# nilsfriess/dune-ddm

Measured on AMD Instinct MI355X. Metric: preconditioned CG iterations/sec (two-level additive Schwarz), 3D Poisson 10M DoF, higher is better.
Workload: dtype f64

## Files before the change

dune-ddm_amd/csrc/kernels.hpp:

```cpp
#pragma once
#include <hip/hip_runtime.h>
#include <stdint.h>

namespace ddm {

constexpr int WG = 256;
constexpr int SPMV_NNZ = 2048;
constexpr int RED_MAX_BLOCKS = 1024;
constexpr int RED_TRIPS = 4;

__device__ __forceinline__ int xcd_remap(int orig, int nwg)
{
  const int q = nwg >> 3, r = nwg & 7, xcd = orig & 7;
  return (xcd < r ? xcd * (q + 1) : r * (q + 1) + (xcd - r) * q) + (orig >> 3);
}

__device__ __forceinline__ double wave_sum(double v)
{
#pragma unroll
  for (int o = 32; o > 0; o >>= 1) v += __shfl_down(v, o, 64);
  return v;
}

__device__ __forceinline__ double block_sum(double v, double *lds4)
// ... 923 lines not shown
    }
    if (stamp) {
      asm volatile("s_waitcnt vmcnt(0)" ::: "memory");
      DDM_STAMP(t_gather)
    }
    const double out = upper ? s * s0 : s;
    if (act) {
      if (wt) st_sc1(x + row, out);
      else x[row] = out;
    }
    if (H.level_done) {
      asm volatile("s_waitcnt vmcnt(0)" ::: "memory");
      if (lane == 0) {
        unsigned *f = flags + H.flag_base + rank;
        if (wt) __hip_atomic_store(f, epoch, __ATOMIC_RELAXED, __HIP_MEMORY_SCOPE_AGENT);
        else *(volatile unsigned *)f = epoch;
      }
    }
    DDM_STAMP(t_drain)
    n_items += 1;
  }
  if (stamp && lane == 0) {
    stamps[0] = t_tile;
    stamps[1] = t_poll;
    stamps[2] = t_gather;
    stamps[3] = t_drain;
    stamps[4] = n_items;
    stamps[5] = __builtin_amdgcn_s_memtime() - t_begin;
  }
#undef DDM_STAMP
}

__global__ void k_w_permute_in(int64_t n, const int64_t *__restrict__ lpos, const int32_t *__restrict__ rows, const double *__restrict__ d,
                               double *__restrict__ dperm)
{
  for (int64_t i = blockIdx.x * (int64_t)WG + threadIdx.x; i < n; i += (int64_t)gridDim.x * WG) dperm[lpos[i]] = d[rows[lpos[i]]];
}
__global__ void k_w_permute_out(int64_t n, const int64_t *__restrict__ upos, const int32_t *__restrict__ rows, const double *__restrict__ xp,
                                double *__restrict__ x)
{
  for (int64_t i = blockIdx.x * (int64_t)WG + threadIdx.x; i < n; i += (int64_t)gridDim.x * WG) x[rows[upos[i]]] = xp[upos[i]];
}

__global__ void k_perm_gather(int64_t n, int nrhs, const int32_t *__restrict__ perm, const double *__restrict__ src, int64_t ld, double *__restrict__ dst)
{
  const int64_t tot = n * nrhs;
  for (int64_t t = blockIdx.x * (int64_t)WG + threadIdx.x; t < tot; t += (int64_t)gridDim.x * WG) {
    const int64_t i = t / nrhs;
    dst[t] = src[(int64_t)perm[i] * ld + (t - i * nrhs)];
  }
}
__global__ void k_perm_scatter(int64_t n, int nrhs, const int32_t *__restrict__ perm, const double *__restrict__ src, double *__restrict__ dst, int64_t ld)
{
  const int64_t tot = n * nrhs;
  for (int64_t t = blockIdx.x * (int64_t)WG + threadIdx.x; t < tot; t += (int64_t)gridDim.x * WG) {
    const int64_t i = t / nrhs;
    dst[(int64_t)perm[i] * ld + (t - i * nrhs)] = src[t];
  }
}
__global__ void k_perm_scatter_add(int64_t n, int nrhs, const int32_t *__restrict__ perm, const double *__restrict__ src, double *__restrict__ dst, int64_t ld)
{
  const int64_t tot = n * nrhs;
  for (int64_t t = blockIdx.x * (int64_t)WG + threadIdx.x; t < tot; t += (int64_t)gridDim.x * WG) {
    const int64_t i = t / nrhs;
    dst[(int64_t)perm[i] * ld + (t - i * nrhs)] += src[t];
  }
}
__global__ __launch_bounds__(WG) void k_residual_rowmajor(int64_t n, int nrhs, const int64_t *__restrict__ rp, const int32_t *__restrict__ ci, const double *__restrict__ va,
                                                          const double *__restrict__ x, int64_t ldx, const double *__restrict__ d, int64_t ldd, double *__restrict__ r, int64_t ldr)
{
  const int64_t t = (int64_t)blockIdx.x * WG + threadIdx.x;
  const int64_t row = t / nrhs;
  if (row >= n) return;
  const int j = (int)(t - row * nrhs);
  double s = d[row * ldd + j];
  for (int64_t k = rp[row]; k < rp[row + 1]; ++k) s -= va[k] * x[(int64_t)ci[k] * ldx + j];
  r[row * ldr + j] = s;
}
__global__ void k_extend(int64_t n, const int32_t *__restrict__ ext_map, const double *__restrict__ d, double *__restrict__ dov)
{
  for (int64_t i = blockIdx.x * (int64_t)WG + threadIdx.x; i < n; i += (int64_t)gridDim.x * WG) {
    const int32_t m = ext_map[i];
    dov[i] = m >= 0 ? d[m] : 0.0;
  }
}
template <bool ACC, bool SCALE>
__global__ void k_restrict(int64_t n, const int32_t *__restrict__ ext_map, const double *__restrict__ xov,
                           const double *__restrict__ w, double *__restrict__ x)
{
  for (int64_t i = blockIdx.x * (int64_t)WG + threadIdx.x; i < n; i += (int64_t)gridDim.x * WG) {
    const int32_t m = ext_map[i];
    if (m >= 0) {
      const double v = SCALE ? xov[i] * w[i] : xov[i];
      x[m] = ACC ? x[m] + v : v;
    }
  }
}
__global__ void k_scale(int64_t n, const double *__restrict__ w, double *__restrict__ x)
{
  for (int64_t i = blockIdx.x * (int64_t)WG + threadIdx.x; i < n; i += (int64_t)gridDim.x * WG) x[i] *= w[i];
}
__global__ void k_fill(int64_t n, double v, double *__restrict__ x)
{
  for (int64_t i = blockIdx.x * (int64_t)WG + threadIdx.x; i < n; i += (int64_t)gridDim.x * WG) x[i] = v;
}
__global__ void k_axpy(int64_t n, double a, const double *__restrict__ x, double *__restrict__ y)
{
  for (int64_t i = blockIdx.x * (int64_t)WG + threadIdx.x; i < n; i += (int64_t)gridDim.x * WG) y[i] += a * x[i];
}

__global__ void k_axpy_negdev(int64_t n, const double *__restrict__ h, const double *__restrict__ x, double *__restrict__ y)
{
  const double a = h[0];
  for (int64_t i = blockIdx.x * (int64_t)WG + threadIdx.x; i < n; i += (int64_t)gridDim.x * WG) y[i] -= a * x[i];
}
__global__ void k_scal(int64_t n, double a, double *__restrict__ x)
{
  for (int64_t i = blockIdx.x * (int64_t)WG + threadIdx.x; i < n; i += (int64_t)gridDim.x * WG) x[i] *= a;
}

__global__ void k_pack(int64_t n, const int64_t *__restrict__ idx, const double *__restrict__ v, double *__restrict__ buf)
{
  for (int64_t i = blockIdx.x * (int64_t)WG + threadIdx.x; i < n; i += (int64_t)gridDim.x * WG) buf[i] = v[idx[i]];
}
template <bool ADD>
__global__ void k_unpack(int64_t ndst, const int64_t *__restrict__ dst_idx, const int64_t *__restrict__ dst_ptr,
                         const int64_t *__restrict__ src_pos, const double *__restrict__ buf, double *__restrict__ v)
{
  for (int64_t t = blockIdx.x * (int64_t)WG + threadIdx.x; t < ndst; t += (int64_t)gridDim.x * WG) {
    const int64_t i = dst_idx[t];
    double s = ADD ? v[i] : 0.0;
    for (int64_t k = dst_ptr[t]; k < dst_ptr[t + 1]; ++k) s = ADD ? s + buf[src_pos[k]] : buf[src_pos[k]];
    v[i] = s;
  }
}

template <bool MASKED>
__global__ __launch_bounds__(WG) void k_dot_partial(int64_t n, const uint8_t *__restrict__ mask, const double *__restrict__ x,
                                                     const double *__restrict__ y, double *__restrict__ partial)
{
  __shared__ double red[4];
  double s = 0.0;
  const int64_t step = (int64_t)gridDim.x * WG;
  int64_t i = blockIdx.x * (int64_t)WG + threadIdx.x;
  for (; i + (RED_TRIPS - 1) * step < n; i += RED_TRIPS * step) {
    double a[RED_TRIPS], b[RED_TRIPS];
    bool own[RED_TRIPS];
#pragma unroll
    for (int u = 0; u < RED_TRIPS; ++u) a[u] = x[i + u * step], b[u] = y[i + u * step], own[u] = !MASKED || mask[i + u * step];
#pragma unroll
    for (int u = 0; u < RED_TRIPS; ++u)
      if (own[u]) s += a[u] * b[u];
  }
  for (; i < n; i += step)
    if (!MASKED || mask[i]) s += x[i] * y[i];
  s = block_sum(s, red);
  if (threadIdx.x == 0) partial[blockIdx.x] = s;
}
__global__ __launch_bounds__(WG) void k_reduce_final(int nb, const double *__restrict__ partial, double *__restrict__ out)
{
  __shared__ double red[4];
  double s = 0.0;
  for (int i = threadIdx.x; i < nb; i += WG) s += partial[i];
  s = block_sum(s, red);
  if (threadIdx.x == 0) out[0] = s;
}

__global__ void k_cg_lambda(double *scal) { scal[2] = scal[0] / scal[1]; }
__global__ void k_cg_beta(double *scal)
{
  scal[4] = scal[3] / scal[0];
  scal[0] = scal[3];
}
__global__ void k_cg_update(int64_t n, const double *__restrict__ scal, const double *__restrict__ p,
                            const double *__restrict__ q, double *__restrict__ x, double *__restrict__ b)
{
  const double lam = scal[2];
  for (int64_t i = blockIdx.x * (int64_t)WG + threadIdx.x; i < n; i += (int64_t)gridDim.x * WG) {
    x[i] += lam * p[i];
    b[i] -= lam * q[i];
  }
}
template <bool MASKED>
__global__ __launch_bounds__(WG) void k_cg_update_norm(int64_t n, const double *__restrict__ scal, const uint8_t *__restrict__ mask,
                                                        const double *__restrict__ p, const double *__restrict__ q, double *__restrict__ x,
                                                        double *__restrict__ b, double *__restrict__ partial)
{
  __shared__ double red[4];
  const double lam = scal[2];
  double s = 0.0;
  for (int64_t i = blockIdx.x * (int64_t)WG + threadIdx.x; i < n; i += (int64_t)gridDim.x * WG) {
    x[i] += lam * p[i];
    const double bi = b[i] - lam * q[i];
    b[i] = bi;
    if (!MASKED || mask[i]) s += bi * bi;
  }
  s = block_sum(s, red);
  if (threadIdx.x == 0) partial[blockIdx.x] = s;
}
__global__ void k_cg_direction(int64_t n, const double *__restrict__ scal, const double *__restrict__ q, double *__restrict__ p)
{
  const double beta = scal[4];
  for (int64_t i = blockIdx.x * (int64_t)WG + threadIdx.x; i < n; i += (int64_t)gridDim.x * WG) p[i] = beta * p[i] + q[i];
}

static constexpr int COARSE_KMAX = 256;
struct RowChunk {
  int64_t r0, r1;
  int32_t sub, pad;
};
__global__ __launch_bounds__(WG) void k_coarse_restrict_partial(int kmax, int64_t ld, const double *__restrict__ basis,
                                                                 const double *__restrict__ d, const RowChunk *__restrict__ chunks,
                                                                 double *__restrict__ partial , int nchunk)
{
  for (int ch = blockIdx.x; ch < nchunk; ch += gridDim.x) {
  const RowChunk c = chunks[ch];
  const int lane = threadIdx.x & 63, w = threadIdx.x >> 6;
  for (int j = w; j < kmax; j += 4) {
    const double *bj = basis + (int64_t)j * ld;
    double s = 0.0;
    int64_t r = c.r0 + lane;
    for (; r + 7 * 64 < c.r1; r += 8 * 64) {
      double bv[8], dv[8];
#pragma unroll
      for (int u = 0; u < 8; ++u) bv[u] = __builtin_nontemporal_load(bj + r + u * 64);
#pragma unroll
      for (int u = 0; u < 8; ++u) dv[u] = d[r + u * 64];
#pragma unroll
      for (int u = 0; u < 8; ++u) s += bv[u] * dv[u];
    }
    for (; r < c.r1; r += 64) s += bj[r] * d[r];
    s = wave_sum(s);
    if (lane == 0) partial[(int64_t)ch * kmax + j] = s;
  }
  }
}
__global__ __launch_bounds__(WG) void k_coarse_restrict_final(int nsub, int kmax, const int32_t *__restrict__ sub_chunk_ptr,
                                                               const double *__restrict__ partial,
                                                               const int64_t *__restrict__ coarse_index, int64_t K,
                                                               double *__restrict__ d0)
{
  for (int64_t i = threadIdx.x; i < K; i += WG) d0[i] = 0.0;
  __syncthreads();
  for (int t = threadIdx.x; t < nsub * kmax; t += WG) {
    const int s = t / kmax, j = t % kmax;
    const int64_t gi = coarse_index[t];
    if (gi < 0) continue;
    double acc = 0.0;
    for (int c = sub_chunk_ptr[s]; c < sub_chunk_ptr[s + 1]; ++c) acc += partial[(int64_t)c * kmax + j];
    d0[gi] = acc;
  }
}
__global__ __launch_bounds__(WG) void k_dense_mv(int64_t K, const double *__restrict__ M, const double *__restrict__ v,
                                                  double *__restrict__ out)
{
  const int lane = threadIdx.x & 63;
  const int64_t row = blockIdx.x * 4 + (threadIdx.x >> 6);
  if (row >= K) return;
  double s = 0.0;
  for (int64_t c = lane; c < K; c += 64) s += M[row * K + c] * v[c];
  s = wave_sum(s);
  if (lane == 0) out[row] = s;
}
__global__ __launch_bounds__(WG) void k_coarse_prolong(int kmax, int64_t ld, const double *__restrict__ basis,
                                                        const double *__restrict__ x0, const int64_t *__restrict__ coarse_index,
                                                        const RowChunk *__restrict__ chunks, double *__restrict__ xov, int nchunk)
{
  __shared__ double cj[COARSE_KMAX];
  static_assert(COARSE_KMAX <= WG, "one thread per coefficient");
  for (int ch = blockIdx.x; ch < nchunk; ch += gridDim.x) {
  const RowChunk c = chunks[ch];
  __syncthreads();
  if (threadIdx.x < kmax) {
    const int64_t gi = coarse_index[(int64_t)c.sub * kmax + threadIdx.x];
    cj[threadIdx.x] = gi >= 0 ? x0[gi] : 0.0;
  }
  __syncthreads();
  for (int64_t r = c.r0 + threadIdx.x; r < c.r1; r += 2 * WG) {
    const int64_t r2 = r + WG < c.r1 ? r + WG : r;
    double s = 0.0, s2 = 0.0;
    int j = 0;
    for (; j + 4 <= kmax; j += 4) {
      double bv[4], bw[4];
#pragma unroll
      for (int u = 0; u < 4; ++u) bv[u] = __builtin_nontemporal_load(basis + (int64_t)(j + u) * ld + r);
#pragma unroll
      for (int u = 0; u < 4; ++u) bw[u] = __builtin_nontemporal_load(basis + (int64_t)(j + u) * ld + r2);
#pragma unroll
      for (int u = 0; u < 4; ++u) s += cj[j + u] * bv[u];
#pragma unroll
      for (int u = 0; u < 4; ++u) s2 += cj[j + u] * bw[u];
    }
    for (; j < kmax; ++j) {
      s += cj[j] * basis[(int64_t)j * ld + r];
      s2 += cj[j] * basis[(int64_t)j * ld + r2];
    }
    xov[r] = s;
    if (r2 != r) xov[r2] = s2;
  }
  }
}

constexpr int SPREAD_WG = 64;
typedef const __attribute__((address_space(1))) double *uniform_gptr;
__device__ __forceinline__ uniform_gptr uniform_global(const double *p)
{
  const uint64_t v = (uint64_t)p;
  const uint32_t lo = __builtin_amdgcn_readfirstlane((uint32_t)v), hi = __builtin_amdgcn_readfirstlane((uint32_t)(v >> 32));
  return (uniform_gptr)(((uint64_t)hi << 32) | lo);
}
__global__ __launch_bounds__(SPREAD_WG) void k_coarse_restrict_spread(int kmax, int64_t ld, const double *__restrict__ basis,
                                                                       const double *__restrict__ d, const RowChunk *__restrict__ chunks,
                                                                       double *__restrict__ partial , int nchunk)
{
  const int lane = threadIdx.x;
  const int64_t nitem = (int64_t)nchunk * kmax;
  for (int64_t item = blockIdx.x; item < nitem; item += gridDim.x) {
    const int ch = (int)(item / kmax), j = (int)(item % kmax);
    const RowChunk c = chunks[ch];
    const double *bj = basis + (int64_t)j * ld;
    double s = 0.0;
    int64_t r = c.r0 + lane;
    for (; r + 7 * 64 < c.r1; r += 8 * 64) {
      double bv[8], dv[8];
#pragma unroll
      for (int u = 0; u < 8; ++u) bv[u] = __builtin_nontemporal_load(bj + r + u * 64);
#pragma unroll
      for (int u = 0; u < 8; ++u) dv[u] = d[r + u * 64];
#pragma unroll
      for (int u = 0; u < 8; ++u) s += bv[u] * dv[u];
    }
    for (; r < c.r1; r += 64) s += bj[r] * d[r];
    s = wave_sum(s);
    if (lane == 0) partial[item] = s;
  }
}
__global__ __launch_bounds__(SPREAD_WG) void k_coarse_prolong_spread(int kmax, int64_t ld, const double *__restrict__ basis,
                                                                      const double *__restrict__ x0, const int64_t *__restrict__ coarse_index,
                                                                      const RowChunk *__restrict__ chunks, double *__restrict__ xov, int nchunk)
{
  __shared__ double cj[COARSE_KMAX];
  const int lane = threadIdx.x;
  for (int ch = blockIdx.x; ch < nchunk; ch += gridDim.x) {
    const RowChunk c = chunks[ch];
    __syncthreads();
    for (int j = lane; j < kmax; j += SPREAD_WG) {
      const int64_t gi = coarse_index[(int64_t)c.sub * kmax + j];
      cj[j] = gi >= 0 ? x0[gi] : 0.0;
    }
    __syncthreads();
    for (int64_t rb = c.r0; rb < c.r1; rb += 4 * SPREAD_WG) {
      const int nrow = (int)(c.r1 - rb < 4 * SPREAD_WG ? c.r1 - rb : 4 * SPREAD_WG);
      if (lane >= nrow) continue;
      unsigned lo[4];
#pragma unroll
      for (int q = 0; q < 4; ++q) lo[q] = (unsigned)(lane + q * SPREAD_WG < nrow ? lane + q * SPREAD_WG : lane);
      double s[4] = {0.0, 0.0, 0.0, 0.0};
      int j = 0;
#pragma unroll 1
      for (; j + 4 <= kmax; j += 4) {
        double bv[4][4];
#pragma unroll
        for (int u = 0; u < 4; ++u) {
          const uniform_gptr bc = uniform_global(basis + (int64_t)(j + u) * ld + rb);
#pragma unroll
          for (int q = 0; q < 4; ++q) bv[q][u] = __builtin_nontemporal_load(bc + lo[q]);
        }
#pragma unroll
        for (int q = 0; q < 4; ++q)
#pragma unroll
          for (int u = 0; u < 4; ++u) s[q] += cj[j + u] * bv[q][u];
      }
      for (; j < kmax; ++j) {
        const double *bc = basis + (int64_t)j * ld + rb;
#pragma unroll
        for (int q = 0; q < 4; ++q) s[q] += cj[j] * bc[lo[q]];
      }
      xov[rb + lo[0]] = s[0];
#pragma unroll
      for (int q = 1; q < 4; ++q)
        if (lo[q] != (unsigned)lane) xov[rb + lo[q]] = s[q];
    }
  }
}

}
```

dune-ddm_amd/csrc/preconditioners.hpp:

```cpp
#pragma once

static int dot_device(ddm_ctx *ctx, int64_t n, const uint8_t *mask, const double *x, const double *y, double *result_dev)
{
  const int nb = grid_for(n, WG * 4, RED_MAX_BLOCKS);
  if (mask)
    hipLaunchKernelGGL(k_dot_partial<true>, dim3(nb), dim3(WG), 0, ctx->stream, n, mask, x, y, ctx->partial);
  else
    hipLaunchKernelGGL(k_dot_partial<false>, dim3(nb), dim3(WG), 0, ctx->stream, n, mask, x, y, ctx->partial);
  hipLaunchKernelGGL(k_reduce_final, dim3(1), dim3(WG), 0, ctx->stream, nb, ctx->partial, result_dev);
  HIPCHECK(ctx, hipGetLastError());
  DDMCHECK(ctx_allreduce(ctx, result_dev, 1, "scalar product"));
  return DDM_OK;
}

template <class Launch>
static void for_column_groups(int m, Launch &&launch)
{
  for (int c0 = 0; c0 < m;) {
    const int cb = m - c0 >= 8 ? 8 : m - c0 >= 4 ? 4 : m - c0 >= 2 ? 2 : 1;
    launch(c0, cb);
    c0 += cb;
  }
}
#define DDM_MULTI_CB_DISPATCH(KERNEL, MASKED, cb, ...)                                                                 \
// ... 197 lines not shown
                  : ddm_ilu0_create(ctx, A_dir, nblocks, block_ptr, &S->solver));
  DDMCHECK(upload(ctx, ext_map_host, n, S->ext_map));
  if (pou_host) DDMCHECK(upload(ctx, pou_host, n, S->pou));
  if (S->d_ovlp.alloc(n) != hipSuccess || S->x_ovlp.alloc(n) != hipSuccess) return fail(ctx, DDM_EHIP, "alloc");
  *out = S.release();
  return DDM_OK;
}
extern "C" void ddm_schwarz_destroy(ddm_schwarz *S) { delete S; }
extern "C" int64_t ddm_schwarz_num_levels(const ddm_schwarz *S, int upper) { return ddm_ilu0_num_levels(S->solver, upper); }
extern "C" int64_t ddm_schwarz_factor_nnz(const ddm_schwarz *S) { return (S && S->solver) ? S->solver->nnz : 0; }
extern "C" int ddm_schwarz_engine(const ddm_schwarz *S) { return S ? ddm_ilu0_engine(S->solver) : -1; }
extern "C" ddm_ilu0 *ddm_schwarz_local_solver(ddm_schwarz *S) { return S ? S->solver : nullptr; }
extern "C" int ddm_schwarz_status(ddm_ctx *ctx, const ddm_schwarz *S)
{
  if (!S) return fail(ctx, DDM_EINVAL, "ddm_schwarz_status: bad arguments");
  int st = 0;
  DDMCHECK(ddm_ilu0_status(ctx, S->solver, &st));
  if (st) return fail(ctx, DDM_ENUMERIC, "local triangular solve timed out waiting for a dependency (code %d): results are invalid", st);
  return DDM_OK;
}
static int local_status_check(ddm_ctx *ctx, const ddm_schwarz *S)
{
  if (const unsigned e = S ? ilu0_peek_status(S->solver) : 0u)
    return fail(ctx, DDM_ENUMERIC, "an earlier local triangular solve timed out waiting for a dependency (code %u): results since then are invalid", e);
  return DDM_OK;
}
static int schwarz_apply_impl(ddm_ctx *ctx, ddm_schwarz *S, double *x, const double *d, bool acc)
{
  DDMCHECK(local_status_check(ctx, S));
  {
    ScopedTimer t(ctx, "Schwarz/get defect");
    hipLaunchKernelGGL(k_extend, dim3(grid_for(S->n)), dim3(WG), 0, ctx->stream, S->n, S->ext_map, d, S->d_ovlp);
    DDMCHECK(ddm_halo_exchange(ctx, S->copy, S->d_ovlp));
  }
  {
    ScopedTimer t(ctx, "Schwarz/local solve");
    DDMCHECK(ddm_ilu0_solve(ctx, S->solver, S->d_ovlp, S->x_ovlp));
  }
  {
    ScopedTimer t(ctx, "Schwarz/add solution");
    if (S->type == 1 && S->pou)
      hipLaunchKernelGGL(k_scale, dim3(grid_for(S->n)), dim3(WG), 0, ctx->stream, S->n, S->pou, S->x_ovlp);
    DDMCHECK(ddm_halo_exchange(ctx, S->add, S->x_ovlp));
    if (acc)
      hipLaunchKernelGGL((k_restrict<true, false>), dim3(grid_for(S->n)), dim3(WG), 0, ctx->stream, S->n, S->ext_map, S->x_ovlp, (const double *)nullptr, x);
    else
      hipLaunchKernelGGL((k_restrict<false, false>), dim3(grid_for(S->n)), dim3(WG), 0, ctx->stream, S->n, S->ext_map, S->x_ovlp, (const double *)nullptr, x);
    HIPCHECK(ctx, hipGetLastError());
  }
  return DDM_OK;
}
extern "C" int ddm_schwarz_apply(ddm_ctx *ctx, ddm_schwarz *S, double *x, const double *d)
{
  ScopedTimer t(ctx, "Schwarz/apply");
  return schwarz_apply_impl(ctx, S, x, d, false);
}
static int schwarz_multi_scratch(ddm_ctx *ctx, ddm_schwarz *S, int m)
{
  HIPCHECK(ctx, reserve_cols<double>(S->mcols, m, {{S->md_ovlp, S->n}, {S->mx_ovlp, S->n}}));
  return DDM_OK;
}
static int schwarz_apply_multi_impl(ddm_ctx *ctx, ddm_schwarz *S, int m, double *X, const double *D, bool acc)
{
  DDMCHECK(local_status_check(ctx, S));
  DDMCHECK(schwarz_multi_scratch(ctx, S, m));
  {
    ScopedTimer t(ctx, "Schwarz/get defect");
    hipLaunchKernelGGL(k_extend_multi, dim3(grid_for(S->n * m)), dim3(WG), 0, ctx->stream, S->n, m, S->ext_map, D, S->md_ovlp);
    DDMCHECK(halo_exchange_multi(ctx, S->copy, m, S->md_ovlp));
  }
  {
    ScopedTimer t(ctx, "Schwarz/local solve");
    DDMCHECK(ilu0_solve_multi_ld(ctx, S->solver, m, S->md_ovlp, m, S->mx_ovlp, m, S->multi_f32));
  }
  {
    ScopedTimer t(ctx, "Schwarz/add solution");
    if (S->type == 1 && S->pou)
      hipLaunchKernelGGL(k_scale_add_multi, dim3(grid_for(S->n * m)), dim3(WG), 0, ctx->stream, S->n, m, (const double *)S->pou, (const double *)nullptr, S->mx_ovlp);
    DDMCHECK(halo_exchange_multi(ctx, S->add, m, S->mx_ovlp));
    if (acc) hipLaunchKernelGGL(k_restrict_multi<true>, dim3(grid_for(S->n * m)), dim3(WG), 0, ctx->stream, S->n, m, S->ext_map, (const double *)S->mx_ovlp, X);
    else hipLaunchKernelGGL(k_restrict_multi<false>, dim3(grid_for(S->n * m)), dim3(WG), 0, ctx->stream, S->n, m, S->ext_map, (const double *)S->mx_ovlp, X);
    HIPCHECK(ctx, hipGetLastError());
  }
  return DDM_OK;
}
extern "C" int ddm_schwarz_apply_multi(ddm_ctx *ctx, ddm_schwarz *S, int nrhs, double *X, const double *D)
{
  if (!ctx || !S || !X || !D || X == D) return fail(ctx, DDM_EINVAL, "ddm_schwarz_apply_multi: bad arguments");
  DDMCHECK(multi_check(ctx, nrhs, "ddm_schwarz_apply_multi"));
  ScopedTimer t(ctx, "Schwarz/apply");
  return schwarz_apply_multi_impl(ctx, S, nrhs, X, D, false);
}
extern "C" int ddm_schwarz_set_multi_precision(ddm_schwarz *S, int f32)
{
  if (!S) return DDM_EINVAL;
  S->multi_f32 = f32 != 0;
  return DDM_OK;
}
extern "C" int ddm_ilu0_set_status(ddm_ilu0 *F, int status)
{
  if (!F || !F->err) return DDM_EINVAL;
  *(volatile unsigned *)F->err = (unsigned)status;
  return DDM_OK;
}

struct ddm_galerkin {
  int64_t n = 0, n_novlp = 0, nsub = 0, kmax = 0, K = 0, ld = 0;
  dbuf<int32_t> ext_map;
  dbuf<double> basis;
  dbuf<int64_t> coarse_index;
  dbuf<double> a0inv;
  dbuf<RowChunk> chunks;
  dbuf<int32_t> sub_chunk_ptr;
  int nchunk = 0;
  dbuf<double> partial, d0, x0;
  dbuf<double> d_ovlp, x_ovlp;
  ddm_halo *copy = nullptr, *add = nullptr;
  dbuf<double> mpartial, md0, mx0, md_ovlp, mx_ovlp;
  int mcols = 0;
};
static constexpr int64_t COARSE_CHUNK_ROWS = 8192;

extern "C" int ddm_galerkin_create(ddm_ctx *ctx, int64_t n, int64_t n_novlp, const int32_t *ext_map_host, int64_t nsub,
                                   const int64_t *sub_ptr, int64_t kmax, const double *basis_host, const int64_t *coarse_index,
                                   int64_t K, const double *a0inv_host, ddm_halo *ovlp_copy, ddm_halo *ovlp_add,
                                   ddm_galerkin **out)
{
  if (!ctx || !out || !ext_map_host || !sub_ptr || !basis_host || !coarse_index || !a0inv_host)
    return fail(ctx, DDM_EINVAL, "ddm_galerkin_create: bad arguments");
  if (kmax < 1) return fail(ctx, DDM_EINVAL, "Must at least pass one template vector");
  if (kmax > COARSE_KMAX) return fail(ctx, DDM_ENOTIMPL, "more than %d basis vectors per subdomain are not supported", COARSE_KMAX);
  if (sub_ptr[0] != 0 || sub_ptr[nsub] != n) return fail(ctx, DDM_EINVAL, "Template vectors must match size of matrix");
  for (int64_t t = 0; t < nsub * kmax; ++t)
    if (coarse_index[t] >= K) return fail(ctx, DDM_EINVAL, "coarse_index out of range");
  auto G = std::make_unique<ddm_galerkin>();
  G->n = n;
  G->n_novlp = n_novlp;
  G->nsub = nsub;
  G->kmax = kmax;
  G->K = K;
  G->ld = (n + 63) / 64 * 64;
  G->copy = ovlp_copy;
  G->add = ovlp_add;
  std::vector<RowChunk> chunks;
  std::vector<int32_t> scp(nsub + 1, 0);
  for (int64_t s = 0; s < nsub; ++s) {
    for (int64_t r = sub_ptr[s]; r < sub_ptr[s + 1]; r += COARSE_CHUNK_ROWS)
      chunks.push_back(RowChunk{r, std::min(r + COARSE_CHUNK_ROWS, sub_ptr[s + 1]), (int32_t)s, 0});
    scp[s + 1] = (int32_t)chunks.size();
  }
  G->nchunk = (int)chunks.size();
  DDMCHECK(upload(ctx, ext_map_host, n, G->ext_map));
  DDMCHECK(upload(ctx, coarse_index, nsub * kmax, G->coarse_index));
  DDMCHECK(upload(ctx, a0inv_host, K * K, G->a0inv));
  DDMCHECK(upload(ctx, chunks.data(), (int64_t)chunks.size(), G->chunks));
  DDMCHECK(upload(ctx, scp.data(), nsub + 1, G->sub_chunk_ptr));
  if (G->basis.alloc(kmax * G->ld) != hipSuccess || G->partial.alloc((int64_t)G->nchunk * kmax) != hipSuccess ||
      G->d0.alloc(K + 1) != hipSuccess ||
      G->x0.alloc(K) != hipSuccess || G->d_ovlp.alloc(n) != hipSuccess || G->x_ovlp.alloc(n) != hipSuccess)
    return fail(ctx, DDM_EHIP, "galerkin: allocation failed");
  if (hipMemset(G->basis, 0, sizeof(double) * (size_t)(kmax * G->ld)) != hipSuccess) return DDM_EHIP;
  if (hipMemcpy2D(G->basis, sizeof(double) * (size_t)G->ld, basis_host, sizeof(double) * (size_t)n, sizeof(double) * (size_t)n,
                  (size_t)kmax, hipMemcpyHostToDevice) != hipSuccess)
    return fail(ctx, DDM_EHIP, "galerkin: basis upload failed");
  *out = G.release();
  return DDM_OK;
}
extern "C" void ddm_galerkin_destroy(ddm_galerkin *G) { delete G; }
static int coarse_chain(ddm_ctx *ctx, ddm_galerkin *G, const double *dov, int spread_grid = 0)
{
  const unsigned sgrid = (unsigned)spread_grid;
  if (spread_grid > 0)
    hipLaunchKernelGGL(k_coarse_restrict_spread, dim3(sgrid), dim3(SPREAD_WG), 0, ctx->stream, (int)G->kmax, G->ld, G->basis, dov, G->chunks, G->partial, G->nchunk);
  else
    hipLaunchKernelGGL(k_coarse_restrict_partial, dim3(G->nchunk), dim3(WG), 0, ctx->stream, (int)G->kmax, G->ld, G->basis, dov, G->chunks, G->partial, G->nchunk);
  hipLaunchKernelGGL(k_coarse_restrict_final, dim3(1), dim3(WG), 0, ctx->stream, (int)G->nsub, (int)G->kmax, G->sub_chunk_ptr, G->partial, G->coarse_index, G->K, G->d0);
  HIPCHECK(ctx, hipGetLastError());
  DDMCHECK(coarse_allreduce(ctx, G->d0, G->K));
  hipLaunchKernelGGL(k_dense_mv, dim3((unsigned)((G->K + 3) / 4)), dim3(WG), 0, ctx->stream, G->K, G->a0inv, G->d0, G->x0);
  if (spread_grid > 0)
    hipLaunchKernelGGL(k_coarse_prolong_spread, dim3(sgrid), dim3(SPREAD_WG), 0, ctx->stream, (int)G->kmax, G->ld, G->basis, G->x0, G->coarse_index, G->chunks, G->x_ovlp, G->nchunk);
  else
    hipLaunchKernelGGL(k_coarse_prolong, dim3(G->nchunk), dim3(WG), 0, ctx->stream, (int)G->kmax, G->ld, G->basis, G->x0, G->coarse_index, G->chunks, G->x_ovlp, G->nchunk);
  return DDM_OK;
}
static int galerkin_apply_impl(ddm_ctx *ctx, ddm_galerkin *G, double *x, const double *d, bool acc, const double *d_ovlp_ready = nullptr)
{
  ScopedTimer t(ctx, "GalerkinPrec/apply");
  const double *dov = d_ovlp_ready;
  if (!dov) {
    hipLaunchKernelGGL(k_extend, dim3(grid_for(G->n)), dim3(WG), 0, ctx->stream, G->n, G->ext_map, d, G->d_ovlp);
    DDMCHECK(ddm_halo_exchange(ctx, G->copy, G->d_ovlp));
    dov = G->d_ovlp;
  }
  DDMCHECK(coarse_chain(ctx, G, dov));
  DDMCHECK(ddm_halo_exchange(ctx, G->add, G->x_ovlp));
  if (acc)
    hipLaunchKernelGGL((k_restrict<true, false>), dim3(grid_for(G->n)), dim3(WG), 0, ctx->stream, G->n, G->ext_map, G->x_ovlp, (const double *)nullptr, x);
  else
    hipLaunchKernelGGL((k_restrict<false, false>), dim3(grid_for(G->n)), dim3(WG), 0, ctx->stream, G->n, G->ext_map, G->x_ovlp, (const double *)nullptr, x);
  HIPCHECK(ctx, hipGetLastError());
  return DDM_OK;
}
extern "C" int ddm_galerkin_apply(ddm_ctx *ctx, ddm_galerkin *G, double *x, const double *d)
{
  return galerkin_apply_impl(ctx, G, x, d, false);
}
extern "C" int ddm_galerkin_debug_chain(ddm_ctx *ctx, ddm_galerkin *G, const double *d_ovlp, int spread_grid, double *partial_out, double *d0_out,
                                        double *x_ovlp_out, int64_t *npartial)
{
  if (!ctx || !G || !npartial || spread_grid < 0) return fail(ctx, DDM_EINVAL, "ddm_galerkin_debug_chain: bad arguments");
  *npartial = (int64_t)G->nchunk * G->kmax;
  if (!partial_out && !d0_out && !x_ovlp_out) return DDM_OK;
  if (!d_ovlp || !partial_out || !d0_out || !x_ovlp_out) return fail(ctx, DDM_EINVAL, "ddm_galerkin_debug_chain: bad arguments");
  DDMCHECK(coarse_chain(ctx, G, d_ovlp, spread_grid));
  HIPCHECK(ctx, hipMemcpyAsync(partial_out, G->partial, sizeof(double) * (size_t)*npartial, hipMemcpyDeviceToDevice, ctx->stream));
  HIPCHECK(ctx, hipMemcpyAsync(d0_out, G->d0, sizeof(double) * (size_t)G->K, hipMemcpyDeviceToDevice, ctx->stream));
  HIPCHECK(ctx, hipMemcpyAsync(x_ovlp_out, G->x_ovlp, sizeof(double) * (size_t)G->n, hipMemcpyDeviceToDevice, ctx->stream));
  HIPCHECK(ctx, hipStreamSynchronize(ctx->stream));
  return DDM_OK;
}
static int galerkin_multi_scratch(ddm_ctx *ctx, ddm_galerkin *G, int m)
{
  HIPCHECK(ctx, reserve_cols<double>(G->mcols, m, {{G->mpartial, (int64_t)G->nchunk * G->kmax}, {G->md0, G->K}, {G->mx0, G->K}, {G->md_ovlp, G->n}, {G->mx_ovlp, G->n}}));
  return DDM_OK;
}
static int coarse_chain_multi(ddm_ctx *ctx, ddm_galerkin *G, int m, const double *dov)
{
  ScopedTimer t(ctx, "GalerkinPrec/apply");
  hipLaunchKernelGGL(k_coarse_restrict_partial_multi, dim3(G->nchunk), dim3(WG), 0, ctx->stream, (int)G->kmax, G->ld, (const double *)G->basis, m, dov,
                     (const RowChunk *)G->chunks, G->mpartial, G->nchunk);
  hipLaunchKernelGGL(k_coarse_restrict_final_multi, dim3(1), dim3(WG), 0, ctx->stream, (int)G->nsub, (int)G->kmax, m, (const int32_t *)G->sub_chunk_ptr,
                     (const double *)G->mpartial, (const int64_t *)G->coarse_index, G->K, G->md0);
  HIPCHECK(ctx, hipGetLastError());
  DDMCHECK(ctx_allreduce(ctx, G->md0, G->K * m, "coarse defect block"));
  if (G->K > 0)
    hipLaunchKernelGGL(k_dense_mm, dim3((unsigned)((G->K * m + WG - 1) / WG)), dim3(WG), 0, ctx->stream, G->K, m, (const double *)G->a0inv, (const double *)G->md0, G->mx0);
  hipLaunchKernelGGL(k_coarse_prolong_multi, dim3(G->nchunk), dim3(WG), 0, ctx->stream, (int)G->kmax, G->ld, (const double *)G->basis, m, (const double *)G->mx0,
                     (const int64_t *)G->coarse_index, (const RowChunk *)G->chunks, G->mx_ovlp, G->nchunk);
  HIPCHECK(ctx, hipGetLastError());
  return DDM_OK;
}
static int galerkin_apply_multi_impl(ddm_ctx *ctx, ddm_galerkin *G, int m, double *X, const double *D, bool acc, const double *dov_ready = nullptr)
{
  DDMCHECK(galerkin_multi_scratch(ctx, G, m));
  const double *dov = dov_ready;
  if (!dov) {
    hipLaunchKernelGGL(k_extend_multi, dim3(grid_for(G->n * m)), dim3(WG), 0, ctx->stream, G->n, m, G->ext_map, D, G->md_ovlp);
    DDMCHECK(halo_exchange_multi(ctx, G->copy, m, G->md_ovlp));
    dov = G->md_ovlp;
  }
  DDMCHECK(coarse_chain_multi(ctx, G, m, dov));
  DDMCHECK(halo_exchange_multi(ctx, G->add, m, G->mx_ovlp));
  if (acc) hipLaunchKernelGGL(k_restrict_multi<true>, dim3(grid_for(G->n * m)), dim3(WG), 0, ctx->stream, G->n, m, G->ext_map, (const double *)G->mx_ovlp, X);
  else hipLaunchKernelGGL(k_restrict_multi<false>, dim3(grid_for(G->n * m)), dim3(WG), 0, ctx->stream, G->n, m, G->ext_map, (const double *)G->mx_ovlp, X);
  HIPCHECK(ctx, hipGetLastError());
  return DDM_OK;
}
extern "C" int ddm_galerkin_apply_multi(ddm_ctx *ctx, ddm_galerkin *G, int nrhs, double *X, const double *D)
{
  if (!ctx || !G || !X || !D || X == D) return fail(ctx, DDM_EINVAL, "ddm_galerkin_apply_multi: bad arguments");
  DDMCHECK(multi_check(ctx, nrhs, "ddm_galerkin_apply_multi"));
  return galerkin_apply_multi_impl(ctx, G, nrhs, X, D, false);
}

extern "C" int ddm_galerkin_products(ddm_ctx *ctx, const ddm_csr *A_dir, int64_t nleft, const double *left, int64_t nright,
                                     const double *right, int64_t row0, int64_t row1, double *out_host)
{
  if (!A_dir || !left || !right || !out_host || nleft < 1 || nleft > COARSE_KMAX || nright < 1 || row0 < 0 || row1 > A_dir->nrows || row0 > row1)
    return fail(ctx, DDM_EINVAL, "ddm_galerkin_products: bad arguments");
  if (A_dir->host_only) return fail(ctx, DDM_EINVAL, "the matrix was created without device arrays (ddm_csr_create_host)");
  const int64_t n = A_dir->nrows;
  dbuf<double> y, partial, outd;
  dbuf<RowChunk> chunks;
  std::vector<RowChunk> hc;
  for (int64_t r = row0; r < row1; r += COARSE_CHUNK_ROWS) hc.push_back(RowChunk{r, std::min(r + COARSE_CHUNK_ROWS, row1), 0, 0});
  const int nchunk = (int)hc.size();
  HIPCHECK(ctx, y.alloc(n));
  HIPCHECK(ctx, partial.alloc((int64_t)nchunk * nleft));
  HIPCHECK(ctx, outd.alloc(nleft * nright));
  int rc = upload(ctx, hc.data(), (int64_t)hc.size(), chunks);
  std::vector<int32_t> scp = {0, nchunk};
  std::vector<int64_t> cidx(nleft);
  dbuf<int32_t> d_scp;
  dbuf<int64_t> d_cidx;
  if (!rc) rc = upload(ctx, scp.data(), 2, d_scp);
  for (int64_t j = 0; j < nright && !rc; ++j) {
    if (row1 > row0)
      hipLaunchKernelGGL(k_spmm_rowmajor, dim3((unsigned)((row1 - row0 + WG - 1) / WG)), dim3(WG), 0, ctx->stream, row1 - row0, 1, A_dir->rp + row0, A_dir->ci, A_dir->va,
                         right + j * n, (int64_t)1, y + row0, (int64_t)1);
    if (hipGetLastError() != hipSuccess) rc = fail(ctx, DDM_EHIP, "ddm_galerkin_products: kernel launch failed");
    for (int64_t i = 0; i < nleft; ++i) cidx[i] = i;
    if (!d_cidx) rc = upload(ctx, cidx.data(), nleft, d_cidx);
    if (rc) break;
    if (nchunk > 0)
      hipLaunchKernelGGL(k_coarse_restrict_partial, dim3(nchunk), dim3(WG), 0, ctx->stream, (int)nleft, n, left, y, chunks, partial, nchunk);
    hipLaunchKernelGGL(k_coarse_restrict_final, dim3(1), dim3(WG), 0, ctx->stream, 1, (int)nleft, d_scp, partial, d_cidx, nleft, outd + j * nleft);
  }
  if (!rc) rc = ddm_memcpy_d2h(ctx, out_host, outd, sizeof(double) * (size_t)(nleft * nright));
  return rc;
}

constexpr bool OVERLAP_DEFAULT = true;
constexpr int OVERLAP_WAVES_PER_CU = 1;
struct ddm_combined {
  int mode = 0;
  ddm_op *op = nullptr;
  ddm_schwarz *schwarz = nullptr;
  ddm_galerkin *galerkin = nullptr;
  dbuf<double> dnext;
  int64_t n = 0;
  bool fused = false;
  int overlap = 0;
  int side_grid = 0;
  dbuf<double> mdnext, mp, mq;
  dbuf<double> mxw, mbw;
  dbuf<int64_t> mqueue_tab;
  dbuf<double> mrt, mv, my;
  int mcols = 0, mcg_cols = 0, mqueue_cols = 0, mbicg_cols = 0;
};
extern "C" int ddm_combined_create(ddm_ctx *ctx, int mode, ddm_op *op, ddm_schwarz *schwarz, ddm_galerkin *galerkin, ddm_combined **out)
{
  if (!ctx || !out || !schwarz) return fail(ctx, DDM_EINVAL, "ERROR: No preconditioners added yet");
  if (mode != 0 && mode != 1) return fail(ctx, DDM_ENOTIMPL, "Unknown apply mode in CombinedPreconditioner, use either additive or multiplicative");
  if (mode == 1 && galerkin && !op) return fail(ctx, DDM_EINVAL, "ERROR: ApplyMode is multiplicative but operator A is not provided. Set with `set_op`");
  auto C = std::make_unique<ddm_combined>();
  C->mode = mode;
  C->op = op;
  C->schwarz = schwarz;
  C->galerkin = galerkin;
  C->n = schwarz->n_novlp;
  if (mode == 0 && galerkin) {
    const char *f = std::getenv("DDM_FUSE_LEVELS");
    const char *e = std::getenv("DDM_OVERLAP_COARSE");
    const char *g = std::getenv("DDM_OVERLAP_GRID");
    C->fused = !(f && f[0] == '0') && galerkin->copy == schwarz->copy && galerkin->add == schwarz->add && galerkin->n == schwarz->n && galerkin->n_novlp == schwarz->n_novlp;
    if (C->fused && (ctx->nranks == 1 || ctx->rccl)) C->overlap = e ? (e[0] == '1' ? 1 : 0) : (OVERLAP_DEFAULT ? 2 : 0);
    C->side_grid = g ? std::max(1, std::atoi(g)) : OVERLAP_WAVES_PER_CU * ctx->num_cu;
  }
  if (C->dnext.alloc(C->n) != hipSuccess) return fail(ctx, DDM_EHIP, "combined: allocation failed");
  *out = C.release();
  return DDM_OK;
}
extern "C" int ddm_combined_status(ddm_ctx *ctx, const ddm_combined *C)
{
  if (!C) return fail(ctx, DDM_EINVAL, "ddm_combined_status: bad arguments");
  return C->schwarz ? ddm_schwarz_status(ctx, C->schwarz) : DDM_OK;
}
extern "C" void ddm_combined_destroy(ddm_combined *C) { delete C; }
static int combined_apply_fused(ddm_ctx *ctx, ddm_combined *C, double *x, const double *d)
{
  ddm_schwarz *S = C->schwarz;
  ddm_galerkin *G = C->galerkin;
  bool pipe_engine = false;
  if (C->overlap != 0) DDMCHECK(ilu0_is_pipe(ctx, S->solver, &pipe_engine));
  const bool two_streams = C->overlap == 1 || (C->overlap == 2 && pipe_engine);
  if (two_streams) DDMCHECK(ctx_side_stream(ctx));
  {
    ScopedTimer t(ctx, "Schwarz/get defect");
    hipLaunchKernelGGL(k_extend, dim3(grid_for(S->n)), dim3(WG), 0, ctx->stream, S->n, S->ext_map, d, S->d_ovlp);
    DDMCHECK(ddm_halo_exchange(ctx, S->copy, S->d_ovlp));
  }
  auto timed_chain = [&](int spread_grid) -> int {
    ScopedTimer t(ctx, "GalerkinPrec/apply");
    return coarse_chain(ctx, G, S->d_ovlp, spread_grid);
  };
  if (two_streams) {
    HIPCHECK(ctx, hipEventRecord(ctx->ev_fork, ctx->stream));
    hipStream_t main = ctx->stream;
    HIPCHECK(ctx, hipStreamWaitEvent(ctx->side, ctx->ev_fork, 0));
    ctx->stream = ctx->side;
    const int rc = timed_chain(C->side_grid);
    const hipError_t e = hipEventRecord(ctx->ev_join, ctx->side);
    ctx->stream = main;
    if (rc) return rc;
    if (e != hipSuccess) return fail(ctx, DDM_EHIP, "hipEventRecord failed: %s", hipGetErrorString(e));
  }
  const double *pou = S->type == 1 ? S->pou : nullptr;
  if (!two_streams) DDMCHECK(timed_chain(0));
  const bool fold = !two_streams || pipe_engine;
  {
    ScopedTimer t(ctx, "Schwarz/local solve");
    DDMCHECK(ilu0_solve_epilogue(ctx, S->solver, S->d_ovlp, S->x_ovlp, fold ? pou : nullptr, fold ? (const double *)G->x_ovlp : nullptr,
                                 two_streams && fold ? ctx->ev_join : nullptr));
  }
  {
    ScopedTimer t(ctx, "Schwarz/add solution");
    if (!fold) {
      if (pou) hipLaunchKernelGGL(k_scale, dim3(grid_for(S->n)), dim3(WG), 0, ctx->stream, S->n, pou, S->x_ovlp);
      HIPCHECK(ctx, hipStreamWaitEvent(ctx->stream, ctx->ev_join, 0));
      hipLaunchKernelGGL(k_axpy, dim3(grid_for(S->n)), dim3(WG), 0, ctx->stream, S->n, 1.0, (const double *)G->x_ovlp, S->x_ovlp);
    }
    DDMCHECK(ddm_halo_exchange(ctx, S->add, S->x_ovlp));
    hipLaunchKernelGGL((k_restrict<false, false>), dim3(grid_for(S->n)), dim3(WG), 0, ctx->stream, S->n, S->ext_map, S->x_ovlp, (const double *)nullptr, x);
    HIPCHECK(ctx, hipGetLastError());
  }
  return DDM_OK;
}

extern "C" int ddm_combined_apply(ddm_ctx *ctx, ddm_combined *C, double *x, const double *d)
{
  ScopedTimer t(ctx, "CombinedPreconditioner/apply");
  DDMCHECK(local_status_check(ctx, C->schwarz));
  if (C->mode == 0 && C->galerkin && C->fused) return combined_apply_fused(ctx, C, x, d);
  DDMCHECK(schwarz_apply_impl(ctx, C->schwarz, x, d, false));
  if (!C->galerkin) return DDM_OK;
  if (C->mode == 0) {
    static const bool no_share = std::getenv("DDM_NO_SHARED_DEFECT") != nullptr;
    const bool share = !no_share && C->galerkin->copy == C->schwarz->copy && C->galerkin->n == C->schwarz->n && C->galerkin->n_novlp == C->schwarz->n_novlp;
    return galerkin_apply_impl(ctx, C->galerkin, x, d, true, share ? C->schwarz->d_ovlp : nullptr);
  }
  HIPCHECK(ctx, hipMemcpyAsync(C->dnext, d, sizeof(double) * (size_t)C->n, hipMemcpyDeviceToDevice, ctx->stream));
  DDMCHECK(ddm_op_applyscaleadd(ctx, C->op, -1.0, x, C->dnext));
  return galerkin_apply_impl(ctx, C->galerkin, x, C->dnext, true);
}
static int combined_apply_multi_impl(ddm_ctx *ctx, ddm_combined *C, int m, double *X, const double *D)
{
  ScopedTimer t(ctx, "CombinedPreconditioner/apply");
  ddm_schwarz *S = C->schwarz;
  ddm_galerkin *G = C->galerkin;
  DDMCHECK(local_status_check(ctx, S));
  if (C->mode == 0 && G && C->fused) {
    DDMCHECK(schwarz_multi_scratch(ctx, S, m));
    DDMCHECK(galerkin_multi_scratch(ctx, G, m));
    {
      ScopedTimer t2(ctx, "Schwarz/get defect");
      hipLaunchKernelGGL(k_extend_multi, dim3(grid_for(S->n * m)), dim3(WG), 0, ctx->stream, S->n, m, S->ext_map, D, S->md_ovlp);
      DDMCHECK(halo_exchange_multi(ctx, S->copy, m, S->md_ovlp));
    }
    DDMCHECK(coarse_chain_multi(ctx, G, m, S->md_ovlp));
    {
      ScopedTimer t2(ctx, "Schwarz/local solve");
      DDMCHECK(ilu0_solve_multi_ld(ctx, S->solver, m, S->md_ovlp, m, S->mx_ovlp, m, S->multi_f32));
    }
    {
      ScopedTimer t2(ctx, "Schwarz/add solution");
      const double *pou = S->type == 1 ? S->pou : nullptr;
      hipLaunchKernelGGL(k_scale_add_multi, dim3(grid_for(S->n * m)), dim3(WG), 0, ctx->stream, S->n, m, pou, (const double *)G->mx_ovlp, S->mx_ovlp);
      DDMCHECK(halo_exchange_multi(ctx, S->add, m, S->mx_ovlp));
      hipLaunchKernelGGL(k_restrict_multi<false>, dim3(grid_for(S->n * m)), dim3(WG), 0, ctx->stream, S->n, m, S->ext_map, (const double *)S->mx_ovlp, X);
      HIPCHECK(ctx, hipGetLastError());
    }
    return DDM_OK;
  }
  DDMCHECK(schwarz_apply_multi_impl(ctx, S, m, X, D, false));
  if (!G) return DDM_OK;
  if (C->mode == 0) {
    const bool share = G->copy == S->copy && G->n == S->n && G->n_novlp == S->n_novlp;
    return galerkin_apply_multi_impl(ctx, G, m, X, D, true, share ? S->md_ovlp : nullptr);
  }
  HIPCHECK(ctx, reserve_cols(C->mcols, m, C->mdnext, C->n));
  HIPCHECK(ctx, hipMemcpyAsync(C->mdnext, D, sizeof(double) * (size_t)(C->n * m), hipMemcpyDeviceToDevice, ctx->stream));
  DDMCHECK(op_applyscaleadd_multi(ctx, C->op, m, -1.0, X, C->mdnext));
  return galerkin_apply_multi_impl(ctx, G, m, X, C->mdnext, true);
}
extern "C" int ddm_combined_apply_multi(ddm_ctx *ctx, ddm_combined *C, int nrhs, double *X, const double *D)
{
  if (!ctx || !C || !X || !D || X == D) return fail(ctx, DDM_EINVAL, "ddm_combined_apply_multi: bad arguments");
  DDMCHECK(multi_check(ctx, nrhs, "ddm_combined_apply_multi"));
  return combined_apply_multi_impl(ctx, C, nrhs, X, D);
}
```

Measured before the change: 223.6.

## Batch coarse restriction over basis-column groups to reuse residual loads

```diff
diff --git a/dune-ddm_amd/csrc/kernels.hpp b/dune-ddm_amd/csrc/kernels.hpp
--- a/dune-ddm_amd/csrc/kernels.hpp
+++ b/dune-ddm_amd/csrc/kernels.hpp
@@ -1249,6 +1249,7 @@
 }
 
 constexpr int SPREAD_WG = 64;
+constexpr int SPREAD_GROUP = 8;
 typedef const __attribute__((address_space(1))) double *uniform_gptr;
 __device__ __forceinline__ uniform_gptr uniform_global(const double *p)
 {
@@ -1256,30 +1257,70 @@
   const uint32_t lo = __builtin_amdgcn_readfirstlane((uint32_t)v), hi = __builtin_amdgcn_readfirstlane((uint32_t)(v >> 32));
   return (uniform_gptr)(((uint64_t)hi << 32) | lo);
 }
+constexpr int spread_trip_rows(int nv) { return nv >= 2 ? (16 + nv - 1) / nv : 8; }
+template <int NV, bool FULL>
+__device__ __forceinline__ void restrict_spread_trip(const double *basis, int64_t ld, int j0, const double *d, int64_t rb, int lane, int nrow, double (&acc)[NV])
+{
+  constexpr int T = spread_trip_rows(NV);
+  unsigned lo[T];
+#pragma unroll
+  for (int q = 0; q < T; ++q) lo[q] = (unsigned)(FULL || lane + q * SPREAD_WG < nrow ? lane + q * SPREAD_WG : 0);
+  double dv[T], bv[NV][T];
+  const uniform_gptr dc = uniform_global(d + rb);
+#pragma unroll
+  for (int q = 0; q < T; ++q) dv[q] = dc[lo[q]];
+#pragma unroll
+  for (int v = 0; v < NV; ++v) {
+    const uniform_gptr bc = uniform_global(basis + (int64_t)(j0 + v) * ld + rb);
+#pragma unroll
+    for (int q = 0; q < T; ++q) bv[v][q] = __builtin_nontemporal_load(bc + lo[q]);
+  }
+#pragma unroll
+  for (int v = 0; v < NV; ++v)
+#pragma unroll
+    for (int q = 0; q < T; ++q)
+      if (FULL || lane + q * SPREAD_WG < nrow) acc[v] += bv[v][q] * dv[q];
+}
+template <int NV>
+__device__ __forceinline__ void restrict_spread_item(const double *basis, int64_t ld, int j0, const double *d, const RowChunk c, int lane, double *out)
+{
+  constexpr int ROWS = spread_trip_rows(NV) * SPREAD_WG;
+  double acc[NV];
+#pragma unroll
+  for (int v = 0; v < NV; ++v) acc[v] = 0.0;
+  int64_t rb = c.r0;
+#pragma unroll 1
+  for (; rb + ROWS <= c.r1; rb += ROWS) restrict_spread_trip<NV, true>(basis, ld, j0, d, rb, lane, ROWS, acc);
+  if (rb < c.r1) restrict_spread_trip<NV, false>(basis, ld, j0, d, rb, lane, (int)(c.r1 - rb), acc);
+#pragma unroll
+  for (int v = 0; v < NV; ++v) {
+    const double s = wave_sum(acc[v]);
+    if (lane == 0) out[v] = s;
+  }
+}
 __global__ __launch_bounds__(SPREAD_WG) void k_coarse_restrict_spread(int kmax, int64_t ld, const double *__restrict__ basis,
                                                                        const double *__restrict__ d, const RowChunk *__restrict__ chunks,
                                                                        double *__restrict__ partial , int nchunk)
 {
+  if (kmax <= 0) return;
   const int lane = threadIdx.x;
-  const int64_t nitem = (int64_t)nchunk * kmax;
+  const int ngroup = (kmax + SPREAD_GROUP - 1) / SPREAD_GROUP, base = kmax / ngroup, rem = kmax % ngroup;
+  const int64_t nitem = (int64_t)nchunk * ngroup;
   for (int64_t item = blockIdx.x; item < nitem; item += gridDim.x) {
-    const int ch = (int)(item / kmax), j = (int)(item % kmax);
+    const int ch = (int)(item / ngroup), g = (int)(item % ngroup);
+    const int nv = base + (g < rem ? 1 : 0), j0 = g * base + (g < rem ? g : rem);
     const RowChunk c = chunks[ch];
-    const double *bj = basis + (int64_t)j * ld;
-    double s = 0.0;
-    int64_t r = c.r0 + lane;
-    for (; r + 7 * 64 < c.r1; r += 8 * 64) {
-      double bv[8], dv[8];
-#pragma unroll
-      for (int u = 0; u < 8; ++u) bv[u] = __builtin_nontemporal_load(bj + r + u * 64);
-#pragma unroll
-      for (int u = 0; u < 8; ++u) dv[u] = d[r + u * 64];
-#pragma unroll
-      for (int u = 0; u < 8; ++u) s += bv[u] * dv[u];
-    }
-    for (; r < c.r1; r += 64) s += bj[r] * d[r];
-    s = wave_sum(s);
-    if (lane == 0) partial[item] = s;
+    double *out = partial + (int64_t)ch * kmax + j0;
+    switch (nv) {
+    case 1: restrict_spread_item<1>(basis, ld, j0, d, c, lane, out); break;
+    case 2: restrict_spread_item<2>(basis, ld, j0, d, c, lane, out); break;
+    case 3: restrict_spread_item<3>(basis, ld, j0, d, c, lane, out); break;
+    case 4: restrict_spread_item<4>(basis, ld, j0, d, c, lane, out); break;
+    case 5: restrict_spread_item<5>(basis, ld, j0, d, c, lane, out); break;
+    case 6: restrict_spread_item<6>(basis, ld, j0, d, c, lane, out); break;
+    case 7: restrict_spread_item<7>(basis, ld, j0, d, c, lane, out); break;
+    default: restrict_spread_item<8>(basis, ld, j0, d, c, lane, out); break;
+    }
   }
 }
 __global__ __launch_bounds__(SPREAD_WG) void k_coarse_prolong_spread(int kmax, int64_t ld, const double *__restrict__ basis,
diff --git a/dune-ddm_amd/csrc/preconditioners.hpp b/dune-ddm_amd/csrc/preconditioners.hpp
--- a/dune-ddm_amd/csrc/preconditioners.hpp
+++ b/dune-ddm_amd/csrc/preconditioners.hpp
@@ -523,7 +523,7 @@
 }
 
 constexpr bool OVERLAP_DEFAULT = true;
-constexpr int OVERLAP_WAVES_PER_CU = 1;
+constexpr int OVERLAP_WAVES_PER_8_CUS = 5;
 struct ddm_combined {
   int mode = 0;
   ddm_op *op = nullptr;
@@ -557,7 +557,7 @@
     const char *g = std::getenv("DDM_OVERLAP_GRID");
     C->fused = !(f && f[0] == '0') && galerkin->copy == schwarz->copy && galerkin->add == schwarz->add && galerkin->n == schwarz->n && galerkin->n_novlp == schwarz->n_novlp;
     if (C->fused && (ctx->nranks == 1 || ctx->rccl)) C->overlap = e ? (e[0] == '1' ? 1 : 0) : (OVERLAP_DEFAULT ? 2 : 0);
-    C->side_grid = g ? std::max(1, std::atoi(g)) : OVERLAP_WAVES_PER_CU * ctx->num_cu;
+    C->side_grid = std::max(1, g ? std::atoi(g) : OVERLAP_WAVES_PER_8_CUS * ctx->num_cu / 8);
   }
   if (C->dnext.alloc(C->n) != hipSuccess) return fail(ctx, DDM_EHIP, "combined: allocation failed");
   *out = C.release();
```

New measurement: 224.2, median of 6. Within noise of the previous version (+0.2%).
